# facebookresearch/holo_diffusion

Hardware: AMD Instinct MI355X
Metric: denoise-steps/sec + rendered-rays/sec, 64^3x32 grid @400^2 render (higher is better)
Workload: dtype f32

## Files before the change

holo_diffusion_amd/csrc/kernels_conv.hip:

```cpp
#include <stdio.h>
#include <stdlib.h>

#include "holo_common.h"
#include "holo_kernels.h"

namespace holo {

using namespace conv_tile;

namespace {

constexpr int LDK = 36;

__device__ __forceinline__ float silu_f(float v) { return v / (1.0f + __expf(-v)); }
__device__ __forceinline__ float silu_fast(float v) { return v * holo_rcp(1.0f + __expf(-v)); }

__device__ __forceinline__ float bf16_load(const uint16_t* p) { return __uint_as_float((uint32_t)(*p) << 16); }
__device__ __forceinline__ uint16_t bf16_round(float v) { return (uint16_t)(pack_bf16x2(v, 0.f) & 0xffffu); }
__device__ __forceinline__ float4 ld_act4(const float* base, int64_t idx, int bf) {
  if (bf) {
    const uint2 u = *reinterpret_cast<const uint2*>(reinterpret_cast<const uint16_t*>(base) + idx);
    return make_float4(__uint_as_float(u.x << 16), __uint_as_float(u.x & 0xffff0000u), __uint_as_float(u.y << 16),
                       __uint_as_float(u.y & 0xffff0000u));
  }
  return *reinterpret_cast<const float4*>(base + idx);
}
__device__ __forceinline__ void st_act4(float* base, int64_t idx, const float4& v, int bf) {
  if (bf)
    *reinterpret_cast<uint2*>(reinterpret_cast<uint16_t*>(base) + idx) = make_uint2(pack_bf16x2(v.x, v.y), pack_bf16x2(v.z, v.w));
  else
    *reinterpret_cast<float4*>(base + idx) = v;
}
__device__ __forceinline__ float ld_act1(const float* base, int64_t idx, int bf) {
  return bf ? bf16_load(reinterpret_cast<const uint16_t*>(base) + idx) : base[idx];
}
__device__ __forceinline__ void st_act1(float* base, int64_t idx, float v, int bf) {
  if (bf)
    reinterpret_cast<uint16_t*>(base)[idx] = bf16_round(v);
  else
    base[idx] = v;
}

__device__ inline int64_t wpack_block(int tap, int cc, int slice, int ncc, int nslice) {
  return (((int64_t)tap * ncc + cc) * nslice + slice) * 512;
}

template <int NT>
__global__ __launch_bounds__(256, 2) void conv_igemm_kernel(ConvParams p) {
  constexpr int BN = 32 * NT;
  constexpr int BUF = (BM + BN) * LDK;
  __shared__ __attribute__((aligned(16))) float lds[2 * BUF];

  const int tid = threadIdx.x;
  const int lane = tid & 63;
  const int wave = tid >> 6;
  const int Cin = p.C0 + p.C1;
  const int ncc = (Cin + BK - 1) / BK;
  const int ntaps = p.ksz * p.ksz * p.ksz;
  const int nchunks = ntaps * ncc;
  const int64_t M = (int64_t)p.N * p.OD * p.OH * p.OW;
  const int64_t m0 = (int64_t)blockIdx.x * BM;
  const int n0 = blockIdx.y * BN;
  const int kc_begin = blockIdx.z * p.chunks_per_split;
  int kc_end = kc_begin + p.chunks_per_split;
  if (kc_end > nchunks) kc_end = nchunks;

  const int wncc = p.CinP / BK, wnsl = p.CoutP >> 4;
  const int q = tid & 7;
  const int r0 = tid >> 3;
  int an[4], az[4], ay[4], ax[4];
  bool av[4];
#pragma unroll
  for (int j = 0; j < 4; ++j) {
    int64_t m = m0 + r0 + 32 * j;
    av[j] = m < M;
    if (!av[j]) m = 0;
    int ow = (int)(m % p.OW);
    int64_t t = m / p.OW;
    int oh = (int)(t % p.OH);
    t /= p.OH;
    int od = (int)(t % p.OD);
    an[j] = (int)(t / p.OD);
    az[j] = od * p.stride - p.pad;
    ay[j] = oh * p.stride - p.pad;
    ax[j] = ow * p.stride - p.pad;
  }
  const int SD = p.ups ? (p.ID >> 1) : p.ID;
  const int SH = p.ups ? (p.IH >> 1) : p.IH;
  const int SW = p.ups ? (p.IW >> 1) : p.IW;

  float4 ra[4];
  float4 rb[NT];
  float4 rc01[4], rc23[4];
  unsigned amask = 0;

  auto load_chunk = [&](int kc) {
    const int tap = kc / ncc;
// ... 1472 lines not shown
    for (int tap = 0; tap < 27; ++tap) {
      const float4(&b)[3][NS] = bRing[tap & 3];
      const float4(&hi)[MT] = aHi[tap & 1];
      if (tap + 1 < 27) load_a(aHi[(tap + 1) & 1], 0, tap + 1);
      if (tap + 3 < 27) load_b(bRing[(tap + 3) & 3], cc, tap + 3);
      if (tap == 26 && cc + 1 < cc_end) halo_issue(cc + 1);
      __builtin_amdgcn_sched_barrier(0);
      mfma4(aLo, b[0]);
      __builtin_amdgcn_sched_barrier(0);
      if (tap + 1 < 27) load_a(aLo, 2, tap + 1);
      __builtin_amdgcn_sched_barrier(0);
      mfma4(hi, b[2]);
      mfma4(aMid, b[1]);
      mfma4(aMid, b[0]);
      __builtin_amdgcn_sched_barrier(0);
      if (tap + 1 < 27) load_a(aMid, 1, tap + 1);
      __builtin_amdgcn_sched_barrier(0);
      mfma4(hi, b[1]);
      mfma4(hi, b[0]);
      __builtin_amdgcn_sched_barrier(0);
    }
    __syncthreads();
  }

  const int64_t M = (int64_t)p.N * p.OD * p.OH * p.OW;
  const int64_t tbase = ((((int64_t)n * p.OD + tz0 + wz) * p.OH + ty0) * p.OW + tx0) * p.Cout;
  int off[MT];
#pragma unroll
  for (int t = 0; t < MT; ++t) off[t] = ((2 * wv + t + 4 * (kq >> 1)) * p.OW + 4 * (kq & 1)) * p.Cout;
#pragma unroll
  for (int s2 = 0; s2 < NS; ++s2) {
    const int co = n0 + (2 * wc + s2) * 16 + lj;
    const int coc = co < p.Cout ? co : p.Cout - 1;
    const float bv = (p.nsplit == 1 && p.bias) ? p.bias[coc] : 0.f;
    float ssum = 0.f, ssq = 0.f;
    if (p.nsplit == 1) {
      if (p.residual) {
        const float* rp = p.residual + tbase + coc;
        float res[MT][4];
#pragma unroll
        for (int t = 0; t < MT; ++t)
#pragma unroll
          for (int r = 0; r < 4; ++r) res[t][r] = rp[off[t] + r * p.Cout];
#pragma unroll
        for (int t = 0; t < MT; ++t)
#pragma unroll
          for (int r = 0; r < 4; ++r) acc[t][s2][r] += res[t][r];
      }
      float* op = p.out + tbase + coc;
#pragma unroll
      for (int t = 0; t < MT; ++t)
#pragma unroll
        for (int r = 0; r < 4; ++r) {
          const float v = acc[t][s2][r] + bv;
          if (co < p.Cout) op[off[t] + r * p.Cout] = v;
          ssum += v;
          ssq += v * v;
        }
    } else if (co < p.Cout) {
      float* pp = p.partial + (int64_t)blockIdx.z * M * p.Cout + tbase + co;
#pragma unroll
      for (int t = 0; t < MT; ++t)
#pragma unroll
        for (int r = 0; r < 4; ++r) pp[off[t] + r * p.Cout] = acc[t][s2][r];
    }
    if (p.stats && p.nsplit == 1) {
      ssum += __shfl_xor(ssum, 16);
      ssq += __shfl_xor(ssq, 16);
      ssum += __shfl_xor(ssum, 32);
      ssq += __shfl_xor(ssq, 32);
      if (kq == 0 && co < p.Cout) {
        const int tiles_per_sample = ntx * nty * ntz;
        const int slab = ((int)(blockIdx.x % tiles_per_sample) * TZ + wz) * 2 + wv;
        double* d = p.stats + (((int64_t)n * tiles_per_sample * TZ * 2 + slab) * p.Cout + co) * 2;
        d[0] = (double)ssum;
        d[1] = (double)ssq;
      }
    }
  }
}

constexpr int SGH = 4;

template <bool BF>
__global__ __launch_bounds__(256, 2) void conv_small_kernel(ConvParams p) {
  constexpr int RW = BF ? 20 : LDK;
  __shared__ __attribute__((aligned(16))) float s_a[SG * SM_ROWS * RW];
  const int tid = threadIdx.x;
  const int lane = tid & 63;
  const int wave = tid >> 6;
  const int lj = lane & 15;
  const int kq = lane >> 4;
  const int Cin = p.C0 + p.C1;
  const int ncc = (Cin + BK - 1) / BK;
  const int ntaps = p.ksz * p.ksz * p.ksz;
  const int SCin = p.skip_w ? p.skip_C0 + p.skip_C1 : 0;
  const int nmain = ntaps * ncc;
  const int nchunks = nmain + (SCin + BK - 1) / BK;
  const int64_t M = (int64_t)p.N * p.OD * p.OH * p.OW;
  const int64_t m0 = (int64_t)blockIdx.x * SM_ROWS;
  const int n0 = blockIdx.y * 64;
  const int kc_begin = blockIdx.z * p.chunks_per_split;
  int kc_end = kc_begin + p.chunks_per_split;
  if (kc_end > nchunks) kc_end = nchunks;

  const int q = tid & 7;
  const int r0 = tid >> 3;
  int an[2], az[2], ay[2], ax[2];
  bool av[2];
#pragma unroll
  for (int j = 0; j < 2; ++j) {
    const int64_t m64 = m0 + r0 + 32 * j;
    av[j] = m64 < M;
    const unsigned m = av[j] ? (unsigned)m64 : 0u;
    int ow = (int)(m % (unsigned)p.OW);
    unsigned t = m / (unsigned)p.OW;
    int oh = (int)(t % (unsigned)p.OH);
    t /= (unsigned)p.OH;
    int od = (int)(t % (unsigned)p.OD);
    an[j] = (int)(t / (unsigned)p.OD);
    az[j] = od * p.stride - p.pad;
    ay[j] = oh * p.stride - p.pad;
    ax[j] = ow * p.stride - p.pad;
  }
  const int SD = p.ups ? (p.ID >> 1) : p.ID;
  const int SH = p.ups ? (p.IH >> 1) : p.IH;
  const int SW = p.ups ? (p.IW >> 1) : p.IW;

  float4 ra[SGH][2], rc01[SGH][2], rc23[SGH][2];
  unsigned amask[SGH];
  int g_tap[SG], g_cc[SG];
  auto load_a = [&](int i, int slot) {
    const int tap = g_tap[slot];
    const int cc = g_cc[slot];
    int kd = 0, kh = 0, kw = 0;
    if (p.ksz == 3) {
      kd = tap / 9;
      kh = (tap - kd * 9) / 3;
      kw = tap - kd * 9 - kh * 3;
    }
    int c = cc * BK + q * 4;
    const bool cvalid = c < Cin;
    if (!cvalid) c = 0;
    const float* src = p.src0;
    int Cs = p.C0, cs = c;
    if (c >= p.C0) {
      src = p.src1;
      Cs = p.C1;
      cs = c - p.C0;
    }
    amask[i] = 0;
#pragma unroll
    for (int j = 0; j < 2; ++j) {
      int z = az[j] + kd, y = ay[j] + kh, x = ax[j] + kw;
      const bool ok = av[j] && cvalid && z >= 0 && z < p.ID && y >= 0 && y < p.IH && x >= 0 && x < p.IW;
      z = min(max(z, 0), p.ID - 1);
      y = min(max(y, 0), p.IH - 1);
      x = min(max(x, 0), p.IW - 1);
      if (p.ups) {
        z >>= 1;
        y >>= 1;
        x >>= 1;
      }
      ra[i][j] = ld_act4(src, ((((int64_t)an[j] * SD + z) * SH + y) * SW + x) * Cs + cs, p.in_bf16);
      amask[i] |= (ok ? 1u : 0u) << j;
      if (p.coef) {
        const float4* cf = reinterpret_cast<const float4*>(p.coef + ((int64_t)an[j] * Cin + c) * 2);
        rc01[i][j] = cf[0];
        rc23[i][j] = cf[1];
      }
    }
  };
  auto store_a = [&](int i, int slot, bool plain = false) {
#pragma unroll
    for (int j = 0; j < 2; ++j) {
      float4 v = ra[i][j];
      if (p.coef && !plain) {
        v.x = v.x * rc01[i][j].x + rc01[i][j].y;
        v.y = v.y * rc01[i][j].z + rc01[i][j].w;
        v.z = v.z * rc23[i][j].x + rc23[i][j].y;
        v.w = v.w * rc23[i][j].z + rc23[i][j].w;
        if (p.act) {
          v.x = silu_f(v.x);
          v.y = silu_f(v.y);
          v.z = silu_f(v.z);
          v.w = silu_f(v.w);
        }
      }
      const float keep = ((amask[i] >> j) & 1u) ? 1.f : 0.f;
      v.x *= keep;
      v.y *= keep;
      v.z *= keep;
      v.w *= keep;
      if (BF)
        *reinterpret_cast<uint2*>(s_a + slot * (SM_ROWS * RW) + (r0 + 32 * j) * RW + q * 2) =
            make_uint2(pack_bf16x2(v.x, v.y), pack_bf16x2(v.z, v.w));
      else
        *reinterpret_cast<float4*>(s_a + slot * (SM_ROWS * RW) + (r0 + 32 * j) * RW + q * 4) = v;
    }
  };

  f32x4 acc[4];
#pragma unroll
  for (int t = 0; t < 4; ++t)
#pragma unroll
    for (int r = 0; r < 4; ++r) acc[t][r] = 0.f;

  const int wncc = p.CinP / BK, wnsl = p.CoutP >> 4;
  constexpr int WBLK = BF ? 256 : 512;
  const float* w_lane = (BF ? reinterpret_cast<const float*>(p.w_bf) : p.w) + (int64_t)((n0 >> 4) + wave) * WBLK + lane * 4;

  const int kc_main_end = kc_end < nmain ? kc_end : nmain;
  auto group_chunks = [&](int g0) {
    int tap = p.ksz == 1 ? 0 : g0 / ncc, cc = g0 - tap * ncc;
#pragma unroll
    for (int i = 0; i < SG; ++i) {
      g_tap[i] = tap, g_cc[i] = cc;
      if (g0 + i + 1 < kc_main_end) {
        ++cc;
        if (cc == ncc) cc = 0, ++tap;
      }
    }
  };
  auto mfma_group = [&](int g, int kend, const float4 (&bw)[SG][2]) {
#pragma unroll
    for (int i = 0; i < SG; ++i) {
      if (g + i < kend) {
        const float* ab = s_a + i * (SM_ROWS * RW) + lj * RW + kq * (BF ? 4 : 8);
        float4 a0[4], a1[4];
#pragma unroll
        for (int t = 0; t < 4; ++t) {
          a0[t] = *reinterpret_cast<const float4*>(ab + t * 16 * RW);
          if (!BF) a1[t] = *reinterpret_cast<const float4*>(ab + t * 16 * RW + 4);
        }
        if (BF) {
#pragma unroll
          for (int t = 0; t < 4; ++t) acc[t] = mfma_bf16_16x16x32(a0[t], bw[i][0], acc[t]);
          continue;
        }
#pragma unroll
        for (int t = 0; t < 4; ++t) acc[t] = __builtin_amdgcn_mfma_f32_16x16x4f32(a0[t].x, bw[i][0].x, acc[t], 0, 0, 0);
#pragma unroll
        for (int t = 0; t < 4; ++t) acc[t] = __builtin_amdgcn_mfma_f32_16x16x4f32(a0[t].y, bw[i][0].y, acc[t], 0, 0, 0);
#pragma unroll
        for (int t = 0; t < 4; ++t) acc[t] = __builtin_amdgcn_mfma_f32_16x16x4f32(a0[t].z, bw[i][0].z, acc[t], 0, 0, 0);
#pragma unroll
        for (int t = 0; t < 4; ++t) acc[t] = __builtin_amdgcn_mfma_f32_16x16x4f32(a0[t].w, bw[i][0].w, acc[t], 0, 0, 0);
#pragma unroll
        for (int t = 0; t < 4; ++t) acc[t] = __builtin_amdgcn_mfma_f32_16x16x4f32(a1[t].x, bw[i][1].x, acc[t], 0, 0, 0);
#pragma unroll
        for (int t = 0; t < 4; ++t) acc[t] = __builtin_amdgcn_mfma_f32_16x16x4f32(a1[t].y, bw[i][1].y, acc[t], 0, 0, 0);
#pragma unroll
        for (int t = 0; t < 4; ++t) acc[t] = __builtin_amdgcn_mfma_f32_16x16x4f32(a1[t].z, bw[i][1].z, acc[t], 0, 0, 0);
#pragma unroll
        for (int t = 0; t < 4; ++t) acc[t] = __builtin_amdgcn_mfma_f32_16x16x4f32(a1[t].w, bw[i][1].w, acc[t], 0, 0, 0);
      }
    }
  };
  for (int g = kc_begin; g < kc_main_end; g += SG) {
    if (g != kc_begin) __syncthreads();
    group_chunks(g);
    float4 bw[SG][2];
    auto load_w = [&]() {
#pragma unroll
      for (int i = 0; i < SG; ++i) {
        const float* wp = w_lane + (int64_t)(g_tap[i] * wncc + g_cc[i]) * wnsl * WBLK;
        bw[i][0] = *reinterpret_cast<const float4*>(wp);
        if (!BF) bw[i][1] = *reinterpret_cast<const float4*>(wp + 256);
      }
    };
#pragma unroll
    for (int h = 0; h < SG; h += SGH) {
      if (g + h < kc_main_end) {
#pragma unroll
        for (int i = 0; i < SGH; ++i) load_a(i, h + i);
        if (!BF && (h + SGH >= SG || g + h + SGH >= kc_main_end)) load_w();
#pragma unroll
        for (int i = 0; i < SGH; ++i) store_a(i, h + i);
      }
    }
    if (BF) load_w();
    __syncthreads();
    mfma_group(g, kc_main_end, bw);
  }
  if (!BF && kc_end > nmain) {
    const float* skw_lane = (BF ? reinterpret_cast<const float*>(p.skip_w_bf) : p.skip_w) + (int64_t)((n0 >> 4) + wave) * WBLK + lane * 4;
    const int sk_lo = (kc_begin > nmain ? kc_begin : nmain) - nmain, sk_hi = kc_end - nmain;
    for (int g = sk_lo; g < sk_hi; g += SG) {
      if (g != sk_lo || kc_begin < nmain) __syncthreads();
      float4 bw[SG][2];
#pragma unroll
      for (int h = 0; h < SG; h += SGH) {
        if (g + h < sk_hi) {
#pragma unroll
          for (int i = 0; i < SGH; ++i) {
            const int sc = g + h + i < sk_hi ? g + h + i : sk_hi - 1;
            int c = sc * BK + q * 4;
            const bool cvalid = c < SCin;
            if (!cvalid) c = 0;
            const float* src = p.skip_src0;
            int Cs = p.skip_C0, cs = c;
            if (c >= p.skip_C0) {
              src = p.skip_src1;
              Cs = p.skip_C1;
              cs = c - p.skip_C0;
            }
            amask[i] = 0;
#pragma unroll
            for (int j = 0; j < 2; ++j) {
              const int z = az[j] + p.pad, y = ay[j] + p.pad, x = ax[j] + p.pad;
              ra[i][j] = ld_act4(src, ((((int64_t)an[j] * p.OD + z) * p.OH + y) * p.OW + x) * Cs + cs, p.in_bf16);
              amask[i] |= (av[j] && cvalid ? 1u : 0u) << j;
            }
          }
          if (h + SGH >= SG || g + h + SGH >= sk_hi) {
#pragma unroll
            for (int i = 0; i < SG; ++i) {
              const int sc = g + i < sk_hi ? g + i : sk_hi - 1;
              const float* wp = skw_lane + (int64_t)sc * wnsl * WBLK;
              bw[i][0] = *reinterpret_cast<const float4*>(wp);
              if (!BF) bw[i][1] = *reinterpret_cast<const float4*>(wp + 256);
            }
          }
#pragma unroll
          for (int i = 0; i < SGH; ++i) store_a(i, h + i, true);
        }
      }
      __syncthreads();
      mfma_group(g, sk_hi, bw);
    }
  }

  const int co = n0 + wave * 16 + lj;
  const int coc = co < p.Cout ? co : p.Cout - 1;
  float bv = (p.nsplit == 1 && p.bias) ? p.bias[coc] : 0.f;
  if (p.nsplit == 1 && p.skip_w && p.skip_bias) bv += p.skip_bias[coc];
  float ssum = 0.f, ssq = 0.f;
  int64_t mo[4][4];
  bool mv[4][4];
#pragma unroll
  for (int t = 0; t < 4; ++t)
#pragma unroll
    for (int r = 0; r < 4; ++r) {
      const int64_t m = m0 + t * 16 + 4 * kq + r;
      mv[t][r] = m < M && co < p.Cout;
      mo[t][r] = (m < M ? m : M - 1) * p.Cout;
    }
  if (p.nsplit == 1) {
    if (p.residual) {
      float res[4][4];
#pragma unroll
      for (int t = 0; t < 4; ++t)
#pragma unroll
        for (int r = 0; r < 4; ++r) res[t][r] = ld_act1(p.residual, mo[t][r] + coc, p.res_bf16);
#pragma unroll
      for (int t = 0; t < 4; ++t)
#pragma unroll
        for (int r = 0; r < 4; ++r) acc[t][r] += res[t][r];
    }
#pragma unroll
    for (int t = 0; t < 4; ++t)
#pragma unroll
      for (int r = 0; r < 4; ++r) {
        const float v = acc[t][r] + bv;
        if (mv[t][r]) {
          st_act1(p.out, mo[t][r] + co, v, p.out_bf16);
          ssum += v;
          ssq += v * v;
        }
      }
  } else {
    float* pp = p.partial + (int64_t)blockIdx.z * M * p.Cout + coc;
#pragma unroll
    for (int t = 0; t < 4; ++t)
#pragma unroll
      for (int r = 0; r < 4; ++r)
        if (mv[t][r]) pp[mo[t][r]] = acc[t][r];
  }
  if (p.stats && p.nsplit == 1) {
    ssum += __shfl_xor(ssum, 16);
    ssq += __shfl_xor(ssq, 16);
    ssum += __shfl_xor(ssum, 32);
    ssq += __shfl_xor(ssq, 32);
    if (kq == 0 && co < p.Cout) {
      const int tiles_per_sample = (int)(((int64_t)p.OD * p.OH * p.OW) / SM_ROWS);
      const int n = (int)(blockIdx.x / tiles_per_sample);
      const int slab = (int)(blockIdx.x % tiles_per_sample);
      double* d = p.stats + (((int64_t)n * tiles_per_sample + slab) * p.Cout + co) * 2;
      d[0] = (double)ssum;
      d[1] = (double)ssq;
    }
  }
}

template <int NCH>
__global__ __launch_bounds__(256, 2) void conv1x1_stream_kernel(ConvParams p) {
  constexpr int DEPTH = NCH <= 4 ? 4 : 2;
  __shared__ __attribute__((aligned(16))) float s_w[NCH * 4 * 2 * 256];
  const int tid = threadIdx.x, lane = tid & 63, wave = tid >> 6, lj = lane & 15, kq = lane >> 4;
  const int64_t M = (int64_t)p.N * p.OD * p.OH * p.OW;
  const int64_t ntile = M >> 4;
  const int n0 = blockIdx.y * 64;
  const int wnsl = p.CoutP >> 4;
  for (int i = tid; i < NCH * 4 * 2 * 64; i += 256) {
    const int ln = i & 63, h = (i >> 6) & 1, sl = (i >> 7) & 3, ch = i >> 9;
    *reinterpret_cast<float4*>(s_w + i * 4) =
        *reinterpret_cast<const float4*>(p.w + ((int64_t)ch * wnsl + (n0 >> 4) + sl) * 512 + h * 256 + ln * 4);
  }
  float4 bv[4];
#pragma unroll
  for (int sl = 0; sl < 4; ++sl)
    bv[sl] = p.bias ? *reinterpret_cast<const float4*>(p.bias + n0 + sl * 16 + 4 * kq) : make_float4(0.f, 0.f, 0.f, 0.f);
  const float* csrc[NCH];
  int cstr[NCH];
#pragma unroll
  for (int i = 0; i < NCH; ++i) {
    const int c = i * 32 + kq * 8;
    const bool second = p.src1 != nullptr && c >= p.C0;
    csrc[i] = (second ? p.src1 + (c - p.C0) : p.src0 + c);
    cstr[i] = second ? p.C1 : p.C0;
  }
  auto load_rows = [&](int64_t t, float4 (&a)[NCH][2]) {
    const int64_t m = t * 16 + lj;
#pragma unroll
    for (int i = 0; i < NCH; ++i) {
      const float* r = csrc[i] + m * cstr[i];
      a[i][0] = *reinterpret_cast<const float4*>(r);
      a[i][1] = *reinterpret_cast<const float4*>(r + 4);
    }
  };
  const int64_t gw = (int64_t)blockIdx.x * 4 + wave, nw = (int64_t)gridDim.x * 4;
  float4 A[DEPTH][NCH][2];
#pragma unroll
  for (int j = 0; j < DEPTH - 1; ++j)
    if (gw + j * nw < ntile) load_rows(gw + j * nw, A[j]);
  __syncthreads();
  for (int64_t t0 = gw; t0 < ntile; t0 += DEPTH * nw) {
#pragma unroll
    for (int j = 0; j < DEPTH; ++j) {
      const int64_t t = t0 + j * nw;
      if (t >= ntile) break;
      if (t + (DEPTH - 1) * nw < ntile) load_rows(t + (DEPTH - 1) * nw, A[(j + DEPTH - 1) % DEPTH]);
      int lw = lane * 4;
      HOLO_LAUNDER(lw);
      const float* wl = s_w + lw;
      f32x4 acc[4];
#pragma unroll
      for (int sl = 0; sl < 4; ++sl)
#pragma unroll
        for (int r = 0; r < 4; ++r) acc[sl][r] = 0.f;
#pragma unroll
      for (int i = 0; i < NCH; ++i)
#pragma unroll
        for (int h = 0; h < 2; ++h) {
          float4 bw[4];
#pragma unroll
          for (int sl = 0; sl < 4; ++sl) bw[sl] = *reinterpret_cast<const float4*>(wl + ((i * 4 + sl) * 2 + h) * 256);
          const float4 a = A[j][i][h];
#pragma unroll
          for (int sl = 0; sl < 4; ++sl) acc[sl] = __builtin_amdgcn_mfma_f32_16x16x4f32(bw[sl].x, a.x, acc[sl], 0, 0, 0);
#pragma unroll
          for (int sl = 0; sl < 4; ++sl) acc[sl] = __builtin_amdgcn_mfma_f32_16x16x4f32(bw[sl].y, a.y, acc[sl], 0, 0, 0);
#pragma unroll
          for (int sl = 0; sl < 4; ++sl) acc[sl] = __builtin_amdgcn_mfma_f32_16x16x4f32(bw[sl].z, a.z, acc[sl], 0, 0, 0);
#pragma unroll
          for (int sl = 0; sl < 4; ++sl) acc[sl] = __builtin_amdgcn_mfma_f32_16x16x4f32(bw[sl].w, a.w, acc[sl], 0, 0, 0);
        }
      float* o = p.out + (t * 16 + lj) * p.Cout + n0 + 4 * kq;
#pragma unroll
      for (int sl = 0; sl < 4; ++sl)
        *reinterpret_cast<float4*>(o + sl * 16) =
            make_float4(acc[sl][0] + bv[sl].x, acc[sl][1] + bv[sl].y, acc[sl][2] + bv[sl].z, acc[sl][3] + bv[sl].w);
    }
  }
}
// ... 212 lines not shown
      dst[e * 2 + 1] = s[4 + e];
    }
  }
}

}

int conv_launch(const ConvParams& p, void* stream) {
  const int Cin = p.C0 + p.C1;
  if (!conv_can_launch(p)) {
    set_error("conv_launch: %s cannot run %d+%d -> %d channels k%d s%d%s @%dx%dx%d batch %d (bf16 %d, storage %d/%d/%d%s%s%s%s), "
              "split-K %d x %d chunks, tz %d, grid_x %d",
              conv_kernel_name(p.kernel), p.C0, p.C1, p.Cout, p.ksz, p.stride, p.ups ? " ups" : "", p.OD, p.OH, p.OW, p.N, p.bf16,
              p.in_bf16, p.out_bf16, p.res_bf16, p.coef ? (p.act ? ", coef+act" : ", coef") : "", p.residual ? ", residual" : "",
              p.skip_w ? ", skip" : "", p.stats ? ", stats" : "", p.nsplit, p.chunks_per_split, p.tz, p.grid_x);
    return -1;
  }
  const int64_t M = (int64_t)p.N * p.OD * p.OH * p.OW;
  const bool wide = p.Cout >= 64;
  const bool sk = p.skip_w != nullptr;
  const int bn = wide ? 64 : 32;
  dim3 block(256);
  dim3 hgrid((unsigned)p.grid_x, (unsigned)cdiv(p.Cout, bn), (unsigned)p.nsplit);
#define HOLO_NCH(KERNEL_, GRID_)                                          \
  switch (Cin / 32) {                                                     \
    case 1: HOLO_LAUNCH(KERNEL_<1>, GRID_, block, stream, p); break;      \
    case 2: HOLO_LAUNCH(KERNEL_<2>, GRID_, block, stream, p); break;      \
    case 3: HOLO_LAUNCH(KERNEL_<3>, GRID_, block, stream, p); break;      \
    case 4: HOLO_LAUNCH(KERNEL_<4>, GRID_, block, stream, p); break;      \
    case 5: HOLO_LAUNCH(KERNEL_<5>, GRID_, block, stream, p); break;      \
    case 6: HOLO_LAUNCH(KERNEL_<6>, GRID_, block, stream, p); break;      \
    case 7: HOLO_LAUNCH(KERNEL_<7>, GRID_, block, stream, p); break;      \
    case 8: HOLO_LAUNCH(KERNEL_<8>, GRID_, block, stream, p); break;      \
    default:                       \
      set_error("conv_launch: no instantiation for %d input channels", Cin); \
      return -1;                                                          \
  }
  switch (p.kernel) {
    case ConvKernel::Gather: {
      dim3 grid((unsigned)cdiv(M, BM), (unsigned)cdiv(p.Cout, bn), (unsigned)p.nsplit);
      if (wide) {
        HOLO_LAUNCH(conv_igemm_kernel<2>, grid, block, stream, p);
      } else {
        HOLO_LAUNCH(conv_igemm_kernel<1>, grid, block, stream, p);
      }
      break;
    }
    case ConvKernel::Halo: {
      if (conv_halo_bf16x3(p)) {
        if (p.tz == 2) {
          HOLO_LAUNCH(conv_halo_split_kernel<2>, hgrid, dim3(512), stream, p);
        } else {
          HOLO_LAUNCH(conv_halo_split_kernel<1>, hgrid, block, stream, p);
        }
        break;
      }
      const bool bf = conv_halo_bf16(p);
#define HOLO_HALO(NWN_, TZ_, SK_)                                                                 \
  do {                                                                                            \
    if (bf) {                                                                                     \
      HOLO_LAUNCH((conv_halo_kernel<NWN_, TZ_, SK_, true>), hgrid, block, stream, p);             \
    } else {                                                                                      \
      HOLO_LAUNCH((conv_halo_kernel<NWN_, TZ_, SK_, false>), hgrid, block, stream, p);            \
    }                                                                                             \
  } while (0)
      if (wide && p.tz == 2 && sk) {
        HOLO_HALO(4, 2, true);
      } else if (wide && p.tz == 2) {
        HOLO_HALO(4, 2, false);
      } else if (wide && sk) {
        HOLO_HALO(4, 1, true);
      } else if (wide) {
        HOLO_HALO(4, 1, false);
      } else if (p.tz == 2) {
        HOLO_HALO(2, 2, false);
      } else {
        HOLO_HALO(2, 1, false);
      }
#undef HOLO_HALO
      break;
    }
    case ConvKernel::RowTile: {
      dim3 sgrid((unsigned)cdiv(M, SM_ROWS), (unsigned)cdiv(p.Cout, 64), (unsigned)p.nsplit);
      if (p.bf16 == 1 && p.w_bf) {
        HOLO_LAUNCH(conv_small_kernel<true>, sgrid, block, stream, p);
      } else {
        HOLO_LAUNCH(conv_small_kernel<false>, sgrid, block, stream, p);
      }
      break;
    }
    case ConvKernel::Wino2:
      if (!wide) {
        HOLO_LAUNCH((conv_wino2_kernel<false, 2>), hgrid, block, stream, p);
      } else if (sk) {
        HOLO_LAUNCH((conv_wino2_kernel<true, 4>), hgrid, block, stream, p);
      } else {
        HOLO_LAUNCH((conv_wino2_kernel<false, 4>), hgrid, block, stream, p);
      }
      break;
    case ConvKernel::Bf16Wide:
      if (!wide) {
        HOLO_LAUNCH((conv_bf16t_kernel<1, false, true>), hgrid, block, stream, p);
      } else if (sk) {
        HOLO_LAUNCH((conv_bf16t_kernel<2, true, true>), hgrid, block, stream, p);
      } else {
        HOLO_LAUNCH((conv_bf16t_kernel<2, false, true>), hgrid, block, stream, p);
      }
      break;
    case ConvKernel::Stream1x1: {
      int64_t wgs = cdiv(M >> 4, 4 * 4);
      if (wgs > 512) wgs = 512;
      if (wgs < 1) wgs = 1;
      dim3 g3((unsigned)wgs, (unsigned)(p.Cout / 64));
      HOLO_NCH(conv1x1_stream_kernel, g3);
      break;
    }
    case ConvKernel::Small1x1: {
      dim3 g1((unsigned)(M / 16), (unsigned)(p.Cout / 64));
      HOLO_NCH(conv1x1_small_kernel, g1);
      break;
    }
    case ConvKernel::Wino3:
      if (conv_wino3_launch(p, stream)) return -1;
      break;
    case ConvKernel::Bf16Persistent: return conv_bf16p_launch(p, stream);
    case ConvKernel::S2Bf16: return conv_s2_bf16_launch(p, stream);
    case ConvKernel::Qkv: return conv1x1_qkv_bf16_launch(p, stream);
    case ConvKernel::Bf16Stream1x1: return conv1x1_bf16_stream_launch(p, stream);
  }
#undef HOLO_NCH
  if (p.nsplit > 1) {
    const int64_t MC = M * p.Cout;
    const int64_t V = (int64_t)p.OD * p.OH * p.OW;
    int B, vpb;
    gn_stats_geometry(p.Cout < 1024 ? p.Cout : 1024, V, &B, &vpb);
    HOLO_LAUNCH(splitk_reduce_kernel, dim3((unsigned)B, (unsigned)p.N, (unsigned)cdiv(p.Cout, 1024)), dim3(256), stream,
                (const float*)p.partial,
                p.nsplit, MC, p.Cout, V, vpb, p.bias, p.skip_bias, p.residual, p.out, p.stats, p.res_bf16, p.out_bf16);
  }
  return 0;
}

}
```

Before: 171.7.

## Specialize row-tile conv kernel with buffer loads and precomputed addressing

Templates the row-tile conv kernel on input dtype, activation mode, upsampling and whole-tile coefficient sharing, and replaces generic per-chunk address math with precomputed row offsets and per-chunk tap offsets read through AMD buffer-resource loads. Bounds masks for the 27 taps are computed once per row, and the per-chunk coefficient reads can be shared per tile. SiLU gets a fast reciprocal-plus-Newton path with a wave-uniform range check, and packed FMA is used for the normalization. It also adds optional timing-probe macros and a host check that rejects inputs past 4 GB, since buffer offsets are 32-bit.

```diff
diff --git a/holo_diffusion_amd/csrc/kernels_conv.hip b/holo_diffusion_amd/csrc/kernels_conv.hip
--- a/holo_diffusion_amd/csrc/kernels_conv.hip
+++ b/holo_diffusion_amd/csrc/kernels_conv.hip
@@ -1,8 +1,11 @@
 #include <stdio.h>
 #include <stdlib.h>
 
+#include <type_traits>
+
 #include "holo_common.h"
 #include "holo_kernels.h"
+#include "rowtile_silu.h"
 
 namespace holo {
 
@@ -12,7 +15,6 @@
 
 constexpr int LDK = 36;
 
-__device__ __forceinline__ float silu_f(float v) { return v / (1.0f + __expf(-v)); }
 __device__ __forceinline__ float silu_fast(float v) { return v * holo_rcp(1.0f + __expf(-v)); }
 
 __device__ __forceinline__ float bf16_load(const uint16_t* p) { return __uint_as_float((uint32_t)(*p) << 16); }
@@ -1651,10 +1653,77 @@
 
 constexpr int SGH = 4;
 
-template <bool BF>
+#ifdef HOLO_EMU
+struct rt_rsrc {
+  const char* base;
+  unsigned n;
+};
+static inline rt_rsrc rt_make_rsrc(const void* p, unsigned nbytes) {
+  return rt_rsrc{reinterpret_cast<const char*>(p), p ? nbytes : 0u};
+}
+static inline float4 rt_ld16(const rt_rsrc& r, unsigned off) {
+  if ((uint64_t)off + 16u > r.n) return make_float4(0.f, 0.f, 0.f, 0.f);
+  return *reinterpret_cast<const float4*>(r.base + off);
+}
+static inline uint2 rt_ld8(const rt_rsrc& r, unsigned off) {
+  if ((uint64_t)off + 8u > r.n) return make_uint2(0u, 0u);
+  return *reinterpret_cast<const uint2*>(r.base + off);
+}
+#define RT_PROBE_BEGIN() ((void)0)
+#define RT_STAMP(k) ((void)0)
+#define RT_WAIT_VM(n) ((void)0)
+#define RT_PROBE_END() ((void)0)
+#else
+typedef __amdgpu_buffer_rsrc_t rt_rsrc;
+typedef unsigned rt_u4 __attribute__((ext_vector_type(4)));
+typedef unsigned rt_u2 __attribute__((ext_vector_type(2)));
+__device__ __forceinline__ rt_rsrc rt_make_rsrc(const void* p, unsigned nbytes) {
+  return __builtin_amdgcn_make_buffer_rsrc(const_cast<void*>(p), 0, p ? nbytes : 0u, 0x00020000);
+}
+__device__ __forceinline__ float4 rt_ld16(rt_rsrc r, unsigned off) {
+  const rt_u4 v = __builtin_amdgcn_raw_buffer_load_b128(r, off, 0, 0);
+  return make_float4(__uint_as_float(v.x), __uint_as_float(v.y), __uint_as_float(v.z), __uint_as_float(v.w));
+}
+__device__ __forceinline__ uint2 rt_ld8(rt_rsrc r, unsigned off) {
+  const rt_u2 v = __builtin_amdgcn_raw_buffer_load_b64(r, off, 0, 0);
+  return make_uint2(v.x, v.y);
+}
+#ifdef HOLO_ROWTILE_PROBE
+#define RT_PROBE_BEGIN()                                                                   \
+  unsigned long long rt_sum[8] = {0, 0, 0, 0, 0, 0, 0, 0}, rt_last;                          \
+  asm volatile("s_memtime %0\n\ts_waitcnt lgkmcnt(0)" : "=s"(rt_last)::"memory")
+#define RT_STAMP(k)                                                                        \
+  do {                                                                                     \
+    __builtin_amdgcn_sched_barrier(0);                                                     \
+    unsigned long long t_;                                                                 \
+    asm volatile("s_memtime %0\n\ts_waitcnt lgkmcnt(0)" : "=s"(t_)::"memory");             \
+    __builtin_amdgcn_sched_barrier(0);                                                     \
+    rt_sum[k] += t_ - rt_last;                                                             \
+    rt_last = t_;                                                                          \
+  } while (0)
+#define RT_WAIT_VM(n) asm volatile("s_waitcnt vmcnt(" #n ")" ::: "memory")
+#define RT_PROBE_END()                                                                                      \
+  do {                                                                                                      \
+    if (p.dbg && threadIdx.x == 0) {                                                                        \
+      unsigned long long* d_ = p.dbg + (((int64_t)blockIdx.z * gridDim.y + blockIdx.y) * gridDim.x + blockIdx.x) * 8; \
+      for (int k_ = 0; k_ < 8; ++k_) d_[k_] = rt_sum[k_];                                                   \
+    }                                                                                                       \
+  } while (0)
+#else
+#define RT_PROBE_BEGIN() ((void)0)
+#define RT_STAMP(k) ((void)0)
+#define RT_WAIT_VM(n) ((void)0)
+#define RT_PROBE_END() ((void)0)
+#endif
+#endif
+
+template <bool BF, bool INBF, int ACTM, bool UPS, bool WHOLE>
 __global__ __launch_bounds__(256, 2) void conv_small_kernel(ConvParams p) {
   constexpr int RW = BF ? 20 : LDK;
+  constexpr unsigned ESZ = INBF ? 2u : 4u;
+  typedef typename std::conditional<INBF, uint2, float4>::type raw4;
   __shared__ __attribute__((aligned(16))) float s_a[SG * SM_ROWS * RW];
+  RT_PROBE_BEGIN();
   const int tid = threadIdx.x;
   const int lane = tid & 63;
   const int wave = tid >> 6;
@@ -1677,11 +1746,16 @@
   const int r0 = tid >> 3;
   int an[2], az[2], ay[2], ax[2];
   bool av[2];
+  unsigned mrow[2], vmask[2], arow0[2], arow1[2], crow[2];
+  const int SD = UPS ? (p.ID >> 1) : p.ID;
+  const int SH = UPS ? (p.IH >> 1) : p.IH;
+  const int SW = UPS ? (p.IW >> 1) : p.IW;
 #pragma unroll
   for (int j = 0; j < 2; ++j) {
     const int64_t m64 = m0 + r0 + 32 * j;
     av[j] = m64 < M;
     const unsigned m = av[j] ? (unsigned)m64 : 0u;
+    mrow[j] = m;
     int ow = (int)(m % (unsigned)p.OW);
     unsigned t = m / (unsigned)p.OW;
     int oh = (int)(t % (unsigned)p.OH);
@@ -1691,82 +1765,120 @@
     az[j] = od * p.stride - p.pad;
     ay[j] = oh * p.stride - p.pad;
     ax[j] = ow * p.stride - p.pad;
-  }
-  const int SD = p.ups ? (p.ID >> 1) : p.ID;
-  const int SH = p.ups ? (p.IH >> 1) : p.IH;
-  const int SW = p.ups ? (p.IW >> 1) : p.IW;
-
-  float4 ra[SGH][2], rc01[SGH][2], rc23[SGH][2];
-  unsigned amask[SGH];
+    unsigned mz = 0, my = 0, mx = 0;
+#pragma unroll
+    for (int k = 0; k < 3; ++k) {
+      mz |= ((unsigned)(az[j] + k) < (unsigned)p.ID ? 1u : 0u) << k;
+      my |= ((unsigned)(ay[j] + k) < (unsigned)p.IH ? 1u : 0u) << k;
+      mx |= ((unsigned)(ax[j] + k) < (unsigned)p.IW ? 1u : 0u) << k;
+    }
+    unsigned m27 = 0;
+#pragma unroll
+    for (int kd = 0; kd < 3; ++kd)
+#pragma unroll
+      for (int kh = 0; kh < 3; ++kh) m27 |= ((mz >> kd) & (my >> kh) & 1u) ? mx << (kd * 9 + kh * 3) : 0u;
+    vmask[j] = av[j] ? m27 : 0u;
+    const unsigned vb = (((unsigned)an[j] * (unsigned)SD + (unsigned)az[j]) * (unsigned)SH + (unsigned)ay[j]) * (unsigned)SW + (unsigned)ax[j];
+    arow0[j] = (vb * (unsigned)p.C0 + (unsigned)q * 4u) * ESZ;
+    arow1[j] = (vb * (unsigned)p.C1 + (unsigned)q * 4u) * ESZ;
+    crow[j] = (unsigned)an[j] * (unsigned)Cin * 8u + (unsigned)q * 32u;
+  }
+  const unsigned ctile = ((unsigned)m0 / ((unsigned)p.OD * (unsigned)p.OH * (unsigned)p.OW)) * (unsigned)Cin * 8u + (unsigned)q * 32u;
+  const rt_rsrc rs0 = rt_make_rsrc(p.src0, (unsigned)p.N * (unsigned)SD * (unsigned)SH * (unsigned)SW * (unsigned)p.C0 * ESZ);
+  const rt_rsrc rs1 = rt_make_rsrc(p.src1, (unsigned)p.N * (unsigned)SD * (unsigned)SH * (unsigned)SW * (unsigned)p.C1 * ESZ);
+  const rt_rsrc rsc = rt_make_rsrc(p.coef, (unsigned)p.N * (unsigned)Cin * 8u);
+
+  raw4 ra[SG][2];
+  float4 rc[SG][2][2];
   int g_tap[SG], g_cc[SG];
-  auto load_a = [&](int i, int slot) {
-    const int tap = g_tap[slot];
-    const int cc = g_cc[slot];
-    int kd = 0, kh = 0, kw = 0;
-    if (p.ksz == 3) {
-      kd = tap / 9;
-      kh = (tap - kd * 9) / 3;
-      kw = tap - kd * 9 - kh * 3;
-    }
-    int c = cc * BK + q * 4;
-    const bool cvalid = c < Cin;
-    if (!cvalid) c = 0;
-    const float* src = p.src0;
-    int Cs = p.C0, cs = c;
-    if (c >= p.C0) {
-      src = p.src1;
-      Cs = p.C1;
-      cs = c - p.C0;
-    }
-    amask[i] = 0;
+  unsigned g_off[SG];
+  bool g_in1[SG];
+  int g_k[SG];
+  auto request = [&](int i, int s, auto pr_c) {
+    constexpr bool PR = decltype(pr_c)::value;
+    const bool in1 = g_in1[s];
+    const rt_rsrc rs = in1 ? rs1 : rs0;
 #pragma unroll
     for (int j = 0; j < 2; ++j) {
-      int z = az[j] + kd, y = ay[j] + kh, x = ax[j] + kw;
-      const bool ok = av[j] && cvalid && z >= 0 && z < p.ID && y >= 0 && y < p.IH && x >= 0 && x < p.IW;
-      z = min(max(z, 0), p.ID - 1);
-      y = min(max(y, 0), p.IH - 1);
-      x = min(max(x, 0), p.IW - 1);
-      if (p.ups) {
-        z >>= 1;
-        y >>= 1;
-        x >>= 1;
-      }
-      ra[i][j] = ld_act4(src, ((((int64_t)an[j] * SD + z) * SH + y) * SW + x) * Cs + cs, p.in_bf16);
-      amask[i] |= (ok ? 1u : 0u) << j;
-      if (p.coef) {
-        const float4* cf = reinterpret_cast<const float4*>(p.coef + ((int64_t)an[j] * Cin + c) * 2);
-        rc01[i][j] = cf[0];
-        rc23[i][j] = cf[1];
-      }
-    }
-  };
-  auto store_a = [&](int i, int slot, bool plain = false) {
+      unsigned vo;
+      if constexpr (UPS) {
+        const int z = (az[j] + (g_k[s] & 3)) >> 1, y = (ay[j] + ((g_k[s] >> 2) & 3)) >> 1, x = (ax[j] + (g_k[s] >> 4)) >> 1;
+        const unsigned vb = (((unsigned)an[j] * (unsigned)SD + (unsigned)z) * (unsigned)SH + (unsigned)y) * (unsigned)SW + (unsigned)x;
+        vo = (vb * (unsigned)(in1 ? p.C1 : p.C0) + (unsigned)q * 4u) * ESZ + g_off[s];
+      } else {
+        vo = (in1 ? arow1[j] : arow0[j]) + g_off[s];
+      }
+      if constexpr (INBF)
+        ra[i][j] = rt_ld8(rs, vo);
+      else
+        ra[i][j] = rt_ld16(rs, vo);
+    }
+    if constexpr (ACTM != 0) {
+      const unsigned co = (unsigned)g_cc[s] * (BK * 8u);
+#pragma unroll
+      for (int j = 0; j < (PR ? 2 : 1); ++j) {
+        rc[i][j][0] = rt_ld16(rsc, (PR ? crow[j] : ctile) + co);
+        rc[i][j][1] = rt_ld16(rsc, (PR ? crow[j] : ctile) + co + 16u);
+      }
+    }
+  };
+  auto commit = [&](int i, int slot, const float (&keep)[2], auto pr_c, auto plain_c) {
+    constexpr bool PR = decltype(pr_c)::value, PLAIN = decltype(plain_c)::value;
+    f32x2 lo[2], hi[2];
 #pragma unroll
     for (int j = 0; j < 2; ++j) {
-      float4 v = ra[i][j];
-      if (p.coef && !plain) {
-        v.x = v.x * rc01[i][j].x + rc01[i][j].y;
-        v.y = v.y * rc01[i][j].z + rc01[i][j].w;
-        v.z = v.z * rc23[i][j].x + rc23[i][j].y;
-        v.w = v.w * rc23[i][j].z + rc23[i][j].w;
-        if (p.act) {
-          v.x = silu_f(v.x);
-          v.y = silu_f(v.y);
-          v.z = silu_f(v.z);
-          v.w = silu_f(v.w);
-        }
-      }
-      const float keep = ((amask[i] >> j) & 1u) ? 1.f : 0.f;
-      v.x *= keep;
-      v.y *= keep;
-      v.z *= keep;
-      v.w *= keep;
-      if (BF)
+      if constexpr (INBF) {
+        const uint2 u = ra[i][j];
+        lo[j] = f32x2{__uint_as_float(u.x << 16), __uint_as_float(u.x & 0xffff0000u)};
+        hi[j] = f32x2{__uint_as_float(u.y << 16), __uint_as_float(u.y & 0xffff0000u)};
+      } else {
+        lo[j] = f32x2{ra[i][j].x, ra[i][j].y};
+        hi[j] = f32x2{ra[i][j].z, ra[i][j].w};
+      }
+      if constexpr (ACTM != 0 && !PLAIN) {
+        const float4 c01 = rc[i][PR ? j : 0][0], c23 = rc[i][PR ? j : 0][1];
+        lo[j] = pk_fma(lo[j], f32x2{c01.x, c01.z}, f32x2{c01.y, c01.w});
+        hi[j] = pk_fma(hi[j], f32x2{c23.x, c23.z}, f32x2{c23.y, c23.w});
+      }
+    }
+    if constexpr (ACTM == 2 && !PLAIN) {
+      float amax = 0.f, amin = SILU_FAST_MAX;
+#pragma unroll
+      for (int j = 0; j < 2; ++j) {
+        amax = fmaxf(fmaxf(fabsf(lo[j].x), fabsf(lo[j].y)), fmaxf(fmaxf(fabsf(hi[j].x), fabsf(hi[j].y)), amax));
+        amin = fminf(fminf(fabsf(lo[j].x), fabsf(lo[j].y)), fminf(fminf(fabsf(hi[j].x), fabsf(hi[j].y)), amin));
+      }
+      if (__builtin_expect(!__any(!(amax <= SILU_FAST_MAX && amin >= SILU_FAST_MIN)), 1)) {
+#pragma unroll
+        for (int j = 0; j < 2; ++j) {
+          lo[j] = f32x2{silu_div_core(lo[j].x, silu_den(lo[j].x)), silu_div_core(lo[j].y, silu_den(lo[j].y))};
+          hi[j] = f32x2{silu_div_core(hi[j].x, silu_den(hi[j].x)), silu_div_core(hi[j].y, silu_den(hi[j].y))};
+        }
+      } else {
+#pragma unroll
+        for (int j = 0; j < 2; ++j) {
+          lo[j] = f32x2{silu_f(lo[j].x), silu_f(lo[j].y)};
+          hi[j] = f32x2{silu_f(hi[j].x), silu_f(hi[j].y)};
+        }
+      }
+    }
+#pragma unroll
+    for (int j = 0; j < 2; ++j) {
+      const f32x2 k2 = f32x2{keep[j], keep[j]};
+      lo[j] = pk_mul(lo[j], k2);
+      hi[j] = pk_mul(hi[j], k2);
+      if constexpr (BF)
         *reinterpret_cast<uint2*>(s_a + slot * (SM_ROWS * RW) + (r0 + 32 * j) * RW + q * 2) =
-            make_uint2(pack_bf16x2(v.x, v.y), pack_bf16x2(v.z, v.w));
+            make_uint2(pack_bf16x2(lo[j].x, lo[j].y), pack_bf16x2(hi[j].x, hi[j].y));
       else
-        *reinterpret_cast<float4*>(s_a + slot * (SM_ROWS * RW) + (r0 + 32 * j) * RW + q * 4) = v;
-    }
+        *reinterpret_cast<float4*>(s_a + slot * (SM_ROWS * RW) + (r0 + 32 * j) * RW + q * 4) =
+            make_float4(lo[j].x, lo[j].y, hi[j].x, hi[j].y);
+    }
+  };
+  auto keep_of = [&](int s, float (&keep)[2]) {
+    const bool cvalid = q * 4 + g_cc[s] * BK < Cin;
+#pragma unroll
+    for (int j = 0; j < 2; ++j) keep[j] = (((vmask[j] >> g_tap[s]) & 1u) != 0u && cvalid) ? 1.f : 0.f;
   };
 
   f32x4 acc[4];
@@ -1777,7 +1889,9 @@
 
   const int wncc = p.CinP / BK, wnsl = p.CoutP >> 4;
   constexpr int WBLK = BF ? 256 : 512;
-  const float* w_lane = (BF ? reinterpret_cast<const float*>(p.w_bf) : p.w) + (int64_t)((n0 >> 4) + wave) * WBLK + lane * 4;
+  const int slice = (n0 >> 4) + HOLO_UNIFORM(wave);
+  const float* w_wave = (BF ? reinterpret_cast<const float*>(p.w_bf) : p.w) + (int64_t)slice * WBLK;
+  const unsigned w_lane = (unsigned)lane * 4u;
 
   const int kc_main_end = kc_end < nmain ? kc_end : nmain;
   auto group_chunks = [&](int g0) {
@@ -1785,6 +1899,19 @@
 #pragma unroll
     for (int i = 0; i < SG; ++i) {
       g_tap[i] = tap, g_cc[i] = cc;
+      {
+        int kd = 0, kh = 0, kw = 0;
+        if (p.ksz == 3) {
+          kd = tap / 9;
+          kh = (tap - kd * 9) / 3;
+          kw = tap - kd * 9 - kh * 3;
+        }
+        const bool in1 = p.src1 != nullptr && cc * BK >= p.C0;
+        const unsigned cs0 = (unsigned)(cc * BK - (in1 ? p.C0 : 0));
+        g_in1[i] = in1;
+        g_k[i] = kd | kh << 2 | kw << 4;
+        g_off[i] = UPS ? cs0 * ESZ : ((unsigned)((kd * p.IH + kh) * p.IW + kw) * (unsigned)(in1 ? p.C1 : p.C0) + cs0) * ESZ;
+      }
       if (g0 + i + 1 < kc_main_end) {
         ++cc;
         if (cc == ncc) cc = 0, ++tap;
@@ -1826,6 +1953,7 @@
       }
     }
   };
+  RT_STAMP(0);
   for (int g = kc_begin; g < kc_main_end; g += SG) {
     if (g != kc_begin) __syncthreads();
     group_chunks(g);
@@ -1833,72 +1961,97 @@
     auto load_w = [&]() {
 #pragma unroll
       for (int i = 0; i < SG; ++i) {
-        const float* wp = w_lane + (int64_t)(g_tap[i] * wncc + g_cc[i]) * wnsl * WBLK;
-        bw[i][0] = *reinterpret_cast<const float4*>(wp);
-        if (!BF) bw[i][1] = *reinterpret_cast<const float4*>(wp + 256);
+        const float* wp = w_wave + (int64_t)(g_tap[i] * wncc + g_cc[i]) * wnsl * WBLK;
+        bw[i][0] = *reinterpret_cast<const float4*>(wp + w_lane);
+        if (!BF) bw[i][1] = *reinterpret_cast<const float4*>(wp + w_lane + 256);
       }
     };
-#pragma unroll
-    for (int h = 0; h < SG; h += SGH) {
-      if (g + h < kc_main_end) {
-#pragma unroll
-        for (int i = 0; i < SGH; ++i) load_a(i, h + i);
-        if (!BF && (h + SGH >= SG || g + h + SGH >= kc_main_end)) load_w();
-#pragma unroll
-        for (int i = 0; i < SGH; ++i) store_a(i, h + i);
-      }
+    auto stage = [&](auto nb_c, auto pr_c, int h, bool with_w) {
+      constexpr int NB = decltype(nb_c)::value;
+#pragma unroll
+      for (int i = 0; i < NB; ++i) request(i, h + i, pr_c);
+      if (with_w) load_w();
+      RT_STAMP(1);
+#ifdef HOLO_ROWTILE_PROBE
+      if (with_w)
+        RT_WAIT_VM(16);
+      else
+        RT_WAIT_VM(0);
+#endif
+      RT_STAMP(2);
+#pragma unroll
+      for (int i = 0; i < NB; ++i) {
+        float keep[2];
+        keep_of(h + i, keep);
+        commit(i, h + i, keep, pr_c, std::false_type());
+      }
+      RT_STAMP(3);
+    };
+    if constexpr (WHOLE) {
+      stage(std::integral_constant<int, SG>(), std::false_type(), 0, true);
+    } else {
+#pragma unroll
+      for (int h = 0; h < SG; h += SGH)
+        if (g + h < kc_main_end)
+          stage(std::integral_constant<int, SGH>(), std::true_type(), h, !BF && (h + SGH >= SG || g + h + SGH >= kc_main_end));
     }
     if (BF) load_w();
     __syncthreads();
+    RT_WAIT_VM(0);
+    RT_STAMP(4);
     mfma_group(g, kc_main_end, bw);
+    RT_STAMP(5);
+#ifdef HOLO_ROWTILE_PROBE
+    rt_sum[7] += 1;
+#endif
   }
   if (!BF && kc_end > nmain) {
-    const float* skw_lane = (BF ? reinterpret_cast<const float*>(p.skip_w_bf) : p.skip_w) + (int64_t)((n0 >> 4) + wave) * WBLK + lane * 4;
+    const float* skw_wave = (BF ? reinterpret_cast<const float*>(p.skip_w_bf) : p.skip_w) + (int64_t)slice * WBLK;
     const int sk_lo = (kc_begin > nmain ? kc_begin : nmain) - nmain, sk_hi = kc_end - nmain;
+    const rt_rsrc rk0 = rt_make_rsrc(p.skip_src0, (unsigned)M * (unsigned)p.skip_C0 * ESZ);
+    const rt_rsrc rk1 = rt_make_rsrc(p.skip_src1, (unsigned)M * (unsigned)p.skip_C1 * ESZ);
+    unsigned krow0[2], krow1[2];
+#pragma unroll
+    for (int j = 0; j < 2; ++j) {
+      krow0[j] = (mrow[j] * (unsigned)p.skip_C0 + (unsigned)q * 4u) * ESZ;
+      krow1[j] = (mrow[j] * (unsigned)p.skip_C1 + (unsigned)q * 4u) * ESZ;
+    }
     for (int g = sk_lo; g < sk_hi; g += SG) {
       if (g != sk_lo || kc_begin < nmain) __syncthreads();
       float4 bw[SG][2];
 #pragma unroll
-      for (int h = 0; h < SG; h += SGH) {
-        if (g + h < sk_hi) {
-#pragma unroll
-          for (int i = 0; i < SGH; ++i) {
-            const int sc = g + h + i < sk_hi ? g + h + i : sk_hi - 1;
-            int c = sc * BK + q * 4;
-            const bool cvalid = c < SCin;
-            if (!cvalid) c = 0;
-            const float* src = p.skip_src0;
-            int Cs = p.skip_C0, cs = c;
-            if (c >= p.skip_C0) {
-              src = p.skip_src1;
-              Cs = p.skip_C1;
-              cs = c - p.skip_C0;
-            }
-            amask[i] = 0;
-#pragma unroll
-            for (int j = 0; j < 2; ++j) {
-              const int z = az[j] + p.pad, y = ay[j] + p.pad, x = ax[j] + p.pad;
-              ra[i][j] = ld_act4(src, ((((int64_t)an[j] * p.OD + z) * p.OH + y) * p.OW + x) * Cs + cs, p.in_bf16);
-              amask[i] |= (av[j] && cvalid ? 1u : 0u) << j;
-            }
-          }
-          if (h + SGH >= SG || g + h + SGH >= sk_hi) {
-#pragma unroll
-            for (int i = 0; i < SG; ++i) {
-              const int sc = g + i < sk_hi ? g + i : sk_hi - 1;
-              const float* wp = skw_lane + (int64_t)sc * wnsl * WBLK;
-              bw[i][0] = *reinterpret_cast<const float4*>(wp);
-              if (!BF) bw[i][1] = *reinterpret_cast<const float4*>(wp + 256);
-            }
-          }
-#pragma unroll
-          for (int i = 0; i < SGH; ++i) store_a(i, h + i, true);
-        }
+      for (int i = 0; i < SG; ++i) {
+        const int sc = g + i < sk_hi ? g + i : sk_hi - 1;
+        const bool in1 = p.skip_src1 != nullptr && sc * BK >= p.skip_C0;
+        const rt_rsrc rs = in1 ? rk1 : rk0;
+        const unsigned so = (unsigned)(sc * BK - (in1 ? p.skip_C0 : 0)) * ESZ;
+#pragma unroll
+        for (int j = 0; j < 2; ++j) {
+          if constexpr (INBF)
+            ra[i][j] = rt_ld8(rs, (in1 ? krow1[j] : krow0[j]) + so);
+          else
+            ra[i][j] = rt_ld16(rs, (in1 ? krow1[j] : krow0[j]) + so);
+        }
+      }
+#pragma unroll
+      for (int i = 0; i < SG; ++i) {
+        const int sc = g + i < sk_hi ? g + i : sk_hi - 1;
+        const float* wp = skw_wave + (int64_t)sc * wnsl * WBLK;
+        bw[i][0] = *reinterpret_cast<const float4*>(wp + w_lane);
+        if (!BF) bw[i][1] = *reinterpret_cast<const float4*>(wp + w_lane + 256);
+      }
+#pragma unroll
+      for (int i = 0; i < SG; ++i) {
+        const int sc = g + i < sk_hi ? g + i : sk_hi - 1;
+        const bool cvalid = q * 4 + sc * BK < SCin;
+        const float keep[2] = {av[0] && cvalid ? 1.f : 0.f, av[1] && cvalid ? 1.f : 0.f};
+        commit(i, i, keep, std::false_type(), std::true_type());
       }
       __syncthreads();
       mfma_group(g, sk_hi, bw);
     }
   }
+  RT_STAMP(5);
 
   const int co = n0 + wave * 16 + lj;
   const int coc = co < p.Cout ? co : p.Cout - 1;
@@ -1960,6 +2113,8 @@
       d[1] = (double)ssq;
     }
   }
+  RT_STAMP(6);
+  RT_PROBE_END();
 }
 
 template <int NCH>
@@ -2338,11 +2493,44 @@
     }
     case ConvKernel::RowTile: {
       dim3 sgrid((unsigned)cdiv(M, SM_ROWS), (unsigned)cdiv(p.Cout, 64), (unsigned)p.nsplit);
+      const int64_t esz = p.in_bf16 ? 2 : 4;
+      const int64_t in_vox = (int64_t)p.N * (p.ID >> (p.ups ? 1 : 0)) * (p.IH >> (p.ups ? 1 : 0)) * (p.IW >> (p.ups ? 1 : 0));
+      const int64_t lim = (int64_t)1 << 32;
+      if (in_vox * (p.C0 > p.C1 ? p.C0 : p.C1) * esz >= lim || (int64_t)p.N * Cin * 8 >= lim ||
+          (p.skip_w && (M * (p.skip_C0 > p.skip_C1 ? p.skip_C0 : p.skip_C1) * esz >= lim || (p.skip_src1 && p.skip_C0 % BK != 0)))) {
+        set_error("conv_launch: conv_small_kernel needs every input within 4 GB (%lld voxels of %d+%d channels) and a fused skip's "
+                  "second source at a multiple of 32 channels (%d+%d)", (long long)in_vox, p.C0, p.C1, p.skip_C0, p.skip_C1);
+        return -1;
+      }
+      const int actm = p.coef ? (p.act ? 2 : 1) : 0;
+      const bool whole = actm == 0 || p.N == 1 || ((int64_t)p.OD * p.OH * p.OW) % SM_ROWS == 0;
+#define HOLO_ROWTILE(BF_, INBF_, W0_, W_)                                                                     \
+  switch (actm * 2 + (p.ups ? 1 : 0)) {                                                                      \
+    case 0: HOLO_LAUNCH((conv_small_kernel<BF_, INBF_, 0, false, W0_>), sgrid, block, stream, p); break;     \
+    case 1: HOLO_LAUNCH((conv_small_kernel<BF_, INBF_, 0, true, W0_>), sgrid, block, stream, p); break;      \
+    case 2: HOLO_LAUNCH((conv_small_kernel<BF_, INBF_, 1, false, W_>), sgrid, block, stream, p); break;      \
+    case 3: HOLO_LAUNCH((conv_small_kernel<BF_, INBF_, 1, true, W_>), sgrid, block, stream, p); break;       \
+    case 4: HOLO_LAUNCH((conv_small_kernel<BF_, INBF_, 2, false, W_>), sgrid, block, stream, p); break;      \
+    default: HOLO_LAUNCH((conv_small_kernel<BF_, INBF_, 2, true, W_>), sgrid, block, stream, p); break;      \
+  }
       if (p.bf16 == 1 && p.w_bf) {
-        HOLO_LAUNCH(conv_small_kernel<true>, sgrid, block, stream, p);
+        if (p.in_bf16) {
+          HOLO_ROWTILE(true, true, false, false)
+        } else {
+          HOLO_ROWTILE(true, false, false, false)
+        }
+      } else if (p.in_bf16) {
+        if (whole) {
+          HOLO_ROWTILE(false, true, true, true)
+        } else {
+          HOLO_ROWTILE(false, true, true, false)
+        }
+      } else if (whole) {
+        HOLO_ROWTILE(false, false, true, true)
       } else {
-        HOLO_LAUNCH(conv_small_kernel<false>, sgrid, block, stream, p);
-      }
+        HOLO_ROWTILE(false, false, true, false)
+      }
+#undef HOLO_ROWTILE
       break;
     }
     case ConvKernel::Wino2:
diff --git a/holo_diffusion_amd/csrc/rowtile_silu.h b/holo_diffusion_amd/csrc/rowtile_silu.h
--- /dev/null
+++ b/holo_diffusion_amd/csrc/rowtile_silu.h
@@ -0,0 +1,28 @@
+#pragma once
+
+#include "holo_common.h"
+
+namespace holo {
+
+constexpr float SILU_FAST_MIN = 8.6736174e-19f;
+constexpr float SILU_FAST_MAX = 64.0f;
+
+__device__ __forceinline__ float silu_den(float v) { return 1.0f + __expf(-v); }
+__device__ __forceinline__ float silu_f(float v) { return v / silu_den(v); }
+
+__device__ __forceinline__ float silu_div_core(float v, float d) {
+#ifdef HOLO_EMU
+  return v / d;
+#else
+  float r = __builtin_amdgcn_rcpf(d);
+  const float e = __builtin_fmaf(-d, r, 1.0f);
+  r = __builtin_fmaf(e, r, r);
+  const float q = v * r;
+  return __builtin_fmaf(__builtin_fmaf(-d, q, v), r, q);
+#endif
+}
+__device__ __forceinline__ bool silu_in_range(float v) {
+  return fmaxf(fabsf(v), 0.f) <= SILU_FAST_MAX && fminf(fabsf(v), SILU_FAST_MAX) >= SILU_FAST_MIN;
+}
+
+}
```

After: 175.2, median of 6. 2.0% higher.
